# tphakala/birda

Hardware: AMD Instinct MI355X
Metric: 3s/48kHz segments/sec (BirdNET v2.4) (higher is better)
Workload: dtype f16x3; 1 GPU; configs[1]: 1000 synthetic 3 s/48 kHz segments per GPU per step, HBM-resident, seeded synthetic BirdNET-v2.4-shaped model (EfficientNet-B0-like, 6522 classes); segments_per_gpu=1000, micro_batch=1000, fused_blocks=16, precision=auto

## Files before the change

### birda_amd/csrc/api.hip

```cpp
#include "api_internal.hpp"
#include <unistd.h>
#include <cerrno>

namespace bhi {


thread_local std::string g_err;

int fail(int code, const char *fmt, ...) {
    char buf[1024];
    va_list ap;
    va_start(ap, fmt);
    vsnprintf(buf, sizeof buf, fmt, ap);
    va_end(ap);
    g_err = buf;
    if (code == BH_ERR_HIP) (void)hipGetLastError();
    return code;
}

int on_exception() noexcept {
    try { throw; }
    catch (const std::bad_alloc &) { return fail(BH_ERR_INTERNAL, "out of host memory"); }
    catch (const std::exception &e) { return fail(BH_ERR_INTERNAL, "internal error: %s", e.what()); }
    catch (...) { return fail(BH_ERR_INTERNAL, "internal error (unknown exception)"); }
// ... 923 lines not shown
        const uint32_t pf = cfg->flags & BH_FLAG_PRECISION_MASK;
        c->precision = pf == BH_FLAG_F32 ? 0 : pf == BH_FLAG_F16 ? 1 : 3;
        c->auto_fallback = pf == BH_FLAG_AUTO;
        c->low_latency = (cfg->flags & BH_FLAG_LOW_LATENCY) != 0;
        c->full_planes = (cfg->flags & BH_FLAG_FULL_PLANES) != 0;
        c->model_path = cfg->model_path;
    }
    if (const char *pe = (cfg->flags & FLAG_INTERNAL_NO_ENV) ? nullptr : getenv("BIRDA_HIP_PRECISION")) {
        if (!strcmp(pe, "f32")) { c->precision = 0; c->auto_fallback = false; }
        else if (!strcmp(pe, "f16x3")) { c->precision = 3; c->auto_fallback = false; }
        else if (!strcmp(pe, "auto")) { c->precision = 3; c->auto_fallback = true; }
        else if (!strcmp(pe, "f16")) { c->precision = 1; c->auto_fallback = false; }
        else return fail(BH_ERR_INVALID, "BIRDA_HIP_PRECISION must be auto, f32, f16x3 or f16");
    }
    int fe_prec = (c->precision != 0 && !(getenv("BIRDA_HIP_MEL_F32") && getenv("BIRDA_HIP_MEL_F32")[0] == '1')) ? 3 : 0;
    for (uint32_t b = 0; b < m.h.n_branches; b++)
        if (m.branches[b].frame_length % 256) fe_prec = 0;
    if (fe_prec == 3) {
        bool want = false, can = true;
        for (uint32_t b = 0; b < m.h.n_branches; b++) {
            if (m.branches[b].frame_step % 16 == 0) want = true;
            if (align_up(m.branches[b].n_mels, 16) % 32 || m.branches[b].frame_length % 512) can = false;
        }
        if (const char *e = getenv("BIRDA_HIP_MEL32")) want = e[0] == '1';
        if (want && can) fe_prec = 32;
    }
    if (m.h.sample_count % 4) return fail(BH_ERR_UNSUPPORTED, "front-end: sample_count %u must be a multiple of 4 (16-byte span loads)", m.h.sample_count);
    c->fe.prec = fe_prec;
    c->fe.n_branches = (int)m.h.n_branches;
    c->fe.sample_count = (int)m.h.sample_count;
    c->fe.norm_eps = m.h.norm_eps;
    for (uint32_t b = 0; b < m.h.n_branches; b++) {
        const auto &br = m.branches[b];
        const int nm_pad = (int)align_up(br.n_mels, 16);
        if (nm_pad < 32 || nm_pad > 128)
            return fail(BH_ERR_UNSUPPORTED, "front-end: n_mels %u not built (17 .. 128)", br.n_mels);
        if (b > 0 && nm_pad != c->fe.br[0].nm_pad) return fail(BH_ERR_UNSUPPORTED, "front-end: branches differ in n_mels");
        if (br.frame_length % 128 || br.fft_length != br.frame_length)
            return fail(BH_ERR_UNSUPPORTED, "front-end: frame_length %u must be a multiple of 128 and equal fft_length", br.frame_length);
        int gf_s = 0;
        std::vector<float> gf = build_gf(br, m.blob.data() + br.mel_w_off, nm_pad, fe_prec, &gf_s);
        float *d = nullptr;
        int rc = upload(gf.data(), gf.size() * sizeof(float), &d);
        if (rc != BH_OK) return rc;
        c->d_owned.push_back(d);
        auto &p = c->fe.br[b];
        p.gf = d; p.L = (int)br.frame_length; p.H = (int)br.frame_step; p.K = p.L / 2;
        p.n_mels = (int)br.n_mels; p.nm_pad = nm_pad; p.n_frames = (int)br.n_frames;
        p.expo = 1.0f / (1.0f + expf(br.mag_scale));
        p.log2_bias = -2.0f * (float)gf_s * p.expo;
        p.out_scale = br.out_scale; p.out_shift = br.out_shift; p.flip = (int)(br.flags & 1u);
        c->mel_flops += 2ull * (uint64_t)p.K * nm_pad * br.n_frames;
    }
    if (bh::mel_lds_bytes(c->fe) > 160 * 1024)
        return fail(BH_ERR_UNSUPPORTED, "front-end: a tile of frames at this hop and frame length spans %zu KB of samples, more than a CU's 160 KB of LDS",
                    bh::mel_lds_bytes(c->fe) / 1024);
    {
        float *d = nullptr;
        int rcf = upload(&c->fe, sizeof c->fe, &d);
        if (rcf != BH_OK) return rcf;
        c->d_fe = reinterpret_cast<bh::FrontendParams *>(d);
        c->d_owned.push_back(d);
    }
    int rc = upload(m.blob.data(), m.blob.size() * sizeof(float), &c->d_blob);
    if (rc != BH_OK) return rc;
    c->d_w.resize(m.layers.size());
    c->ldw.assign(m.layers.size(), 0);
    for (size_t i = 0; i < m.layers.size(); i++) {
        const auto &L = m.layers[i];
        c->d_w[i] = c->d_blob + L.w_off;
        if (L.op == bh::OP_PWCONV || L.op == bh::OP_DENSE) {
            if (L.cin % 4) return fail(BH_ERR_UNSUPPORTED, "layer %zu: cin %u not a multiple of 4", i, L.cin);
            const int ld = (int)align_up(L.cout, 4);
            c->ldw[i] = ld;
            if (ld != (int)L.cout) {
                const std::vector<float> w = pw_gemm_rows(m.blob.data() + L.w_off, L.cin, L.cout, (size_t)ld);
                float *d = nullptr;
                rc = upload(w.data(), w.size() * sizeof(float), &d);
                if (rc != BH_OK) return rc;
                c->d_owned.push_back(d);
                c->d_w[i] = d;
            }
        } else if (L.op == bh::OP_DWCONV) {
            if (!bh::dwconv_supports(conv_params(L)))
                return fail(BH_ERR_UNSUPPORTED, "layer %zu: depthwise %ux%u stride %u channels %u not built", i, L.kh, L.kw, L.sh, L.cout);
        } else if (L.op == bh::OP_CONV && L.in_layout == 1) {
            if (!bh::conv_direct_supports(conv_params(L)))
                return fail(BH_ERR_UNSUPPORTED, "layer %zu: direct conv shape not built", i);
        } else if (L.op == bh::OP_CONV) {
            const bh::ConvParams p = conv_params(L);
            if (!bh::conv_gemm_supports(p))
                return fail(BH_ERR_UNSUPPORTED, "layer %zu: full convolution %ux%u stride %ux%u, %u -> %u channels, layout %u not built "
                            "(kernel 1..7, stride 1 / 2, channels multiples of 4, NHWC)", i, L.kh, L.kw, L.sh, L.sw, L.cin, L.cout, L.in_layout);
            const int ld = (int)align_up(L.cout, 4);
            c->ldw[i] = ld;
            const std::vector<float> w = conv_gemm_rows(m.blob.data() + L.w_off, p, ld);
            float *d = nullptr;
            rc = upload(w.data(), w.size() * sizeof(float), &d);
            if (rc != BH_OK) return rc;
            c->d_owned.push_back(d);
            c->d_w[i] = d;
        } else if (L.op == bh::OP_GCONV) {
            const bh::ConvParams p = conv_params(L);
            if (!bh::gconv_supports(p, (int)L.reserved))
                return fail(BH_ERR_UNSUPPORTED, "layer %zu: grouped convolution %ux%u stride %ux%u, %u -> %u channels in %u groups not built "
                            "(kernel 1..7, stride 1 / 2, group widths multiples of 4, NHWC, no residual)", i, L.kh, L.kw, L.sh, L.sw, L.cin, L.cout, L.reserved);
// ... 1594 lines not shown
```

### birda_amd/csrc/kernels.hpp

```cpp
#pragma once
#include <hip/hip_runtime.h>
#include <stdint.h>

#include <atomic>
#include <cmath>
#include <mutex>

#ifdef BIRDA_HIP_EXPERIMENTS
#define BH_XENV(name) getenv(name)
#else
#define BH_XENV(name) (static_cast<const char *>(nullptr))
#endif

namespace bh {

constexpr int MAX_DEVICES = 64;
inline int current_device() {
    int d = 0;
    if (hipGetDevice(&d) != hipSuccess || d < 0 || d >= MAX_DEVICES) d = 0;
    return d;
}
struct DeviceOnce {
    std::mutex mu;
    std::atomic<unsigned char> done[MAX_DEVICES] = {};
// ... 203 lines not shown
__device__ __forceinline__ float bh_act(float v) {
    if constexpr (ACT == ACT_NONE) return v;
    else if constexpr (ACT == ACT_GELU_ERF) return gelu_erf_fast(v);
    else if constexpr (ACT == ACT_RELU) return bh_relu1(v);
    else if constexpr (ACT == ACT_RELU6) return __builtin_amdgcn_fmed3f(v, 0.0f, 6.0f);
    else if constexpr (ACT == ACT_SWISH) return v * __builtin_amdgcn_rcpf(1.0f + __builtin_amdgcn_exp2f(-1.4426950408889634f * v));
    else return act_apply_slow(v, ACT);
}
template <int ACT>
__device__ __forceinline__ bh_f32x2 bh_act2(bh_f32x2 v) {
    if constexpr (ACT == ACT_GELU_ERF) return gelu_erf_fast2(v);
    else { bh_f32x2 r; r[0] = bh_act<ACT>(v[0]); r[1] = bh_act<ACT>(v[1]); return r; }
}
template <int ACT>
__device__ __forceinline__ void bh_act4(bh_f32x2 &v0, bh_f32x2 &v1) {
    if constexpr (ACT == ACT_GELU_ERF) gelu_erf_fast4(v0, v1);
    else { v0 = bh_act2<ACT>(v0); v1 = bh_act2<ACT>(v1); }
}
inline bool act_is_templated(int act) { return act == ACT_GELU_ERF || act == ACT_SWISH || act == ACT_RELU6; }

__device__ __forceinline__ float bh_relu_keep_nan(float v) { return v < 0.0f ? 0.0f : v; }
__device__ __forceinline__ float bh_relu6_keep_nan(float v) { return v < 0.0f ? 0.0f : (v > 6.0f ? 6.0f : v); }
__device__ __forceinline__ float bh_act_limits(float v, float r) {
    r = v == __builtin_inff() ? v : r;
    return v == -__builtin_inff() ? 0.0f : r;
}
template <int ACT>
__device__ __forceinline__ float bh_act_after(float v) {
    if constexpr (ACT == ACT_RELU) return bh_relu_keep_nan(v);
    else if constexpr (ACT == ACT_RELU6) return bh_relu6_keep_nan(v);
    else return bh_act_limits(v, bh_act<ACT>(v));
}
__device__ __forceinline__ float act_apply_pos(float v, int act, bool after) {
    switch (act) {
    case ACT_RELU: return after ? bh_relu_keep_nan(v) : fmaxf(v, 0.f);
    case ACT_RELU6: return after ? bh_relu6_keep_nan(v) : fminf(fmaxf(v, 0.f), 6.f);
    case ACT_SWISH: { const float r = v / (1.0f + expf(-v)); return after ? bh_act_limits(v, r) : r; }
    case ACT_GELU_ERF: { const float r = gelu_erf_fast(v); return after ? bh_act_limits(v, r) : r; }
    case ACT_GELU_TANH: { const float r = 0.5f * v * (1.0f + tanhf(0.7978845608028654f * (v + 0.044715f * v * v * v))); return after ? bh_act_limits(v, r) : r; }
    case ACT_SIGMOID: return 1.0f / (1.0f + expf(-v));
    default: return v;
    }
}
inline bool act_is_templated_after(int act) { return act == ACT_RELU || act_is_templated(act); }

struct BranchParams {
    const float *gf;
    int L, H, K;
    int n_mels, nm_pad, n_frames;
    float expo;
    float out_scale, out_shift;
    int flip;
    float log2_bias;
};
struct FrontendParams {
    BranchParams br[MAX_BRANCHES];
    int prec;
    int n_branches;
    int sample_count;
    float norm_eps;
};

void launch_segment_pcm(const void *d_pcm_origin, int sample_format, size_t n_frames, int channels, const unsigned long long *d_starts,
                        int n_seg, int seg_len, float *d_out, size_t out_stride, hipStream_t s);
void launch_minmax(const float *x, float *minmax, unsigned *in_bad, int n_seg, int sample_count, hipStream_t s);
size_t mel_lds_bytes(const FrontendParams &p);
const char *launch_mel(const float *x, const float *minmax, float *spec, const FrontendParams &p,
                       const FrontendParams *d_p, int n_seg, hipStream_t s);


struct ConvParams {
    int in_h, in_w, out_h, out_w, cin, cout, kh, kw, sh, sw, pad_t, pad_l, in_layout, act;
    int res_after = 0;
};
bool conv_direct_supports(const ConvParams &p);
const char *launch_conv_direct(const float *in, const float *w, const float *b, float *out, const ConvParams &p,
                        int n_seg, hipStream_t s);
bool conv_gemm_supports(const ConvParams &p);
bool conv_gemm16_supports(const ConvParams &p);
bool conv_gemm16_after_supports(const ConvParams &p);
const char *launch_conv_gemm(const float *in, const float *W, const float *b, const float *R, float *out, const ConvParams &p, int n_seg,
                             int ldw, hipStream_t s);
const char *launch_conv_gemm16(const float *in, const void *Wf, const float *b, const float *R, float *out, const ConvParams &p, int n_seg,
                               int terms, float w_unscale, hipStream_t s);
__host__ __device__ inline void gconv_tile_span(int cin, int cout, int groups, int t, int &c0, int &span) {
    const int gi = cin / groups, go = cout / groups;
    const int last = (16 * t + 15 < cout ? 16 * t + 15 : cout - 1) / go, first = 16 * t / go;
    c0 = first * gi;
    span = (last - first + 1) * gi;
}
bool gconv_supports(const ConvParams &p, int groups);
const char *launch_gconv(const float *in, const float *Wf, const float *b, float *out, const ConvParams &p, int groups, int n_seg, hipStream_t s);
const char *launch_gconv16(const float *in, const void *Wf, const float *b, float *out, const ConvParams &p, int groups, int n_seg, int terms,
                           float w_unscale, hipStream_t s);
bool dwconv_supports(const ConvParams &p);
const char *launch_dwconv(const float *in, const float *w, const float *b, float *out, const ConvParams &p,
                   int n_seg, hipStream_t s);
const char *launch_pw_gemm(const float *A, const float *W, const float *bias, const float *R, float *C, int M, int K,
                          int N, int ldw, int act, hipStream_t s, int res_after = 0);
bool pw_gemm16_supports(int K, int act);
bool pw_gemm16_after_supports(int K, int act);
const char *launch_pw_gemm16(const float *A, const void *Wf, const float *bias, const float *R, float *C, int M, int K, int N,
                             int act, int terms, float w_unscale, hipStream_t s, int res_after = 0);
const char *launch_pw_gemm_gated(const float *A, const float *gate, int rows_per_seg, const float *W, const float *bias, const float *R,
                                 float *C, int M, int K, int N, int ldw, int act, hipStream_t s, int res_after = 0);
bool pw_gemm16_gated_wants_blocked(int K, int N, int rows_per_seg);
const char *launch_pw_gemm16_gated(const float *A, const float *gate, int rows_per_seg, const void *Wf, const float *bias, const float *R,
                                   float *C, int M, int K, int N, int terms, float w_unscale, int a_blocked, hipStream_t s);
bool se_gate16_supports(int C, int Cr);
const char *launch_se_gate16(const float *part, int tiles, int P, float *hpart, const float *W1, const float *b1, int ld1, int act1, const float *W2,
                      const float *b2, int ld2, int act2, float *gate, int n_seg, int C, int Cr, hipStream_t s);
bool se_gate_supports(int C, int Cr);
const char *launch_se_gate_gemm(const float *part, int tiles, int P, float *pooled, float *hidden, const float *W1, const float *b1, int ld1, int act1,
                         const float *W2, const float *b2, int ld2, int act2, float *gate, int n_seg, int C, int Cr, hipStream_t s);
const char *launch_se_gate(const float *part, int tiles, int P, const float *W1, const float *b1, int ld1, int act1, const float *W2, const float *b2,
                    int ld2, int act2, float *gate, int n_seg, int C, int Cr, hipStream_t s);
const char *launch_gap(const float *in, float *out, int n_seg, int P, int C, hipStream_t s);
const char *launch_scale(const float *in, const float *gate, float *out, int n_seg, int P, int C, hipStream_t s);
// ... 68 lines not shown
```

### birda_amd/csrc/kernels_frontend.hip

```cpp
#include <algorithm>
#include <cstdlib>

#include "kernels.hpp"

namespace bh {

constexpr int MM_SPLIT = 8;

typedef float f32x4 __attribute__((ext_vector_type(4)));
typedef _Float16 f16x8 __attribute__((ext_vector_type(8)));

__device__ inline float wave_min(float v) {
#pragma unroll
    for (int o = 32; o > 0; o >>= 1) v = fminf(v, __shfl_xor(v, o, 64));
    return v;
}
__device__ inline float wave_max(float v) {
#pragma unroll
    for (int o = 32; o > 0; o >>= 1) v = fmaxf(v, __shfl_xor(v, o, 64));
    return v;
}

__global__ __launch_bounds__(256) void minmax_kernel(const float *__restrict__ x, float *__restrict__ mm,
                                                      unsigned *__restrict__ in_bad, int sample_count) {
    const int seg = blockIdx.y, part = blockIdx.x;
    const int n4 = sample_count >> 2;
    const int per = (n4 + MM_SPLIT - 1) / MM_SPLIT;
    const int lo = part * per, hi = min(n4, lo + per);
    const float4 *p = reinterpret_cast<const float4 *>(x + (size_t)seg * sample_count);
    float mn = INFINITY, mx = -INFINITY;
    float z0 = 0.0f, z1 = 0.0f;
    for (int i = lo + threadIdx.x; i < hi; i += 256) {
        float4 v = p[i];
        mn = fminf(fminf(mn, v.x), fminf(v.y, fminf(v.z, v.w)));
        mx = fmaxf(fmaxf(mx, v.x), fmaxf(v.y, fmaxf(v.z, v.w)));
        z0 = __builtin_fmaf(v.x, 0.0f, z0); z1 = __builtin_fmaf(v.y, 0.0f, z1);
        z0 = __builtin_fmaf(v.z, 0.0f, z0); z1 = __builtin_fmaf(v.w, 0.0f, z1);
    }
    if (part == MM_SPLIT - 1)
        for (int i = (n4 << 2) + threadIdx.x; i < sample_count; i += 256) {
            float v = x[(size_t)seg * sample_count + i];
            mn = fminf(mn, v); mx = fmaxf(mx, v);
            z0 = __builtin_fmaf(v, 0.0f, z0);
        }
    mn = wave_min(mn); mx = wave_max(mx);
    const int any_bad = __syncthreads_or((z0 + z1) != 0.0f ? 1 : 0);
    __shared__ float s[8];
    const int w = threadIdx.x >> 6;
    if ((threadIdx.x & 63) == 0) { s[w] = mn; s[4 + w] = mx; }
    __syncthreads();
    if (threadIdx.x == 0) {
        mn = fminf(fminf(s[0], s[1]), fminf(s[2], s[3]));
        mx = fmaxf(fmaxf(s[4], s[5]), fmaxf(s[6], s[7]));
        mm[((size_t)seg * MM_SPLIT + part) * 2 + 0] = mn;
// ... 12 lines not shown
    else if constexpr (FMT == 2) {
        const int32_t v = (int32_t)((uint32_t)p[0] << 8 | (uint32_t)p[1] << 16 | (uint32_t)p[2] << 24);
        return (float)v / 2147483648.0f;
    } else if constexpr (FMT == 3) return (float)*reinterpret_cast<const int32_t *>(p) / 2147483648.0f;
    else return *reinterpret_cast<const float *>(p);
}

template <int FMT>
__global__ __launch_bounds__(256) void segment_pcm_kernel(const unsigned char *__restrict__ pcm, long n_frames, int channels,
                                                           const unsigned long long *__restrict__ starts,
                                                           int seg_len, float *__restrict__ out, long out_stride) {
    constexpr int BPS = FMT == 1 ? 2 : FMT == 2 ? 3 : 4;
    const int seg = blockIdx.y;
    const long s0 = (long)starts[seg];
    float *o = out + (long)seg * out_stride;
    for (int j = blockIdx.x * 256 + threadIdx.x; j < seg_len; j += gridDim.x * 256) {
        const long f = s0 + j;
        float v = 0.0f;
        if (f < n_frames) {
            if (channels == 1) {
                v = pcm_sample<FMT>(pcm + f * BPS);
            } else {
                float sum = 0.0f;
                for (int c = 0; c < channels; c++) sum += pcm_sample<FMT>(pcm + (f * channels + c) * BPS);
                v = sum / (float)channels;
            }
        }
        o[j] = v;
    }
}

void launch_segment_pcm(const void *d_pcm_origin, int sample_format, size_t n_frames, int channels, const unsigned long long *d_starts,
                        int n_seg, int seg_len, float *d_out, size_t out_stride, hipStream_t s) {
    dim3 grid((unsigned)std::min<size_t>(((size_t)seg_len + 255) / 256, 64), n_seg), block(256);
    const unsigned char *p = static_cast<const unsigned char *>(d_pcm_origin);
#define BH_SEG(F) hipLaunchKernelGGL(segment_pcm_kernel<F>, grid, block, 0, s, p, (long)n_frames, channels, d_starts, seg_len, d_out, (long)out_stride)
    switch (sample_format) {
    case 2: BH_SEG(2); break;
    case 3: BH_SEG(3); break;
    case 4: BH_SEG(4); break;
    default: BH_SEG(1); break;
    }
#undef BH_SEG
}

#ifndef BH_MEL_PIPE
#define BH_MEL_PIPE 2
#endif
#ifndef BH_MEL_GM
#define BH_MEL_GM 6
#define BH_MEL_GD 6
#define BH_MEL_GV 8
#endif
constexpr int MEL_FT = 3;
constexpr int MEL_TN = 16 * MEL_FT;


template <int MT, int PREC, int HALVES = 1>
__global__ __launch_bounds__(256 * HALVES, (MT <= 6 || HALVES == 2) ? 2 : 1) void mel_kernel(const float *__restrict__ x, const float *__restrict__ mm,
                                                      float *__restrict__ spec, const FrontendParams *__restrict__ pp,
                                                      const float *__restrict__ gf0, const float *__restrict__ gf1,
                                                      const float *__restrict__ gf2, const float *__restrict__ gf3,
                                                      const int dbg_arg, const int n_tiles, const int n_items, const int paired) {
    extern __shared__ __attribute__((aligned(16))) float smem[];
#ifdef BIRDA_HIP_EXPERIMENTS
    const int dbg = dbg_arg;
#else
    constexpr int dbg = 0; (void)dbg_arg;
#endif
    const int n_branches = pp->n_branches;
    const int S = pp->sample_count;
    float *xs = smem;
    const int tid = threadIdx.x, lane = tid & 63;
    const int half = HALVES == 2 ? tid >> 8 : 0, wave = (tid >> 6) & 3;
    const int li = lane & 15, kq = lane >> 4;
    constexpr int TNW = MEL_TN * HALVES, NTHR = 256 * HALVES;

    static_assert(MM_SPLIT == 8, "16 floats of min / max partials per segment");
    constexpr int MEL_SU = HALVES == 2 ? 14 : (MT <= 6 ? 15 : 16);
    float4 q[MEL_SU], mmq[4];
    const int pr_xcd = blockIdx.x & 7, pr_slot = blockIdx.x >> 3;
    const int pr_role = paired ? pr_slot % n_branches : 0, pr_q = (pr_slot / n_branches) * 8 + pr_xcd;
    const int pr_stride = (int)gridDim.x / n_branches, n_pairs = n_items / n_branches;
    struct MelItem { int sg, br, tl, ok; };
    auto decode = [&](int n) __attribute__((always_inline)) -> MelItem {
        MelItem r;
        if (paired) {
            const int P = pr_q + n * pr_stride;
            r.br = (pr_role + n) % n_branches;
            r.sg = P / n_tiles; r.tl = P - r.sg * n_tiles;
            r.ok = P < n_pairs;
        } else {
            const int it = (int)blockIdx.x + n * (int)gridDim.x;
            r.tl = it % n_tiles;
            const int sb = it / n_tiles;
            r.sg = sb / n_branches; r.br = sb - r.sg * n_branches;
            r.ok = it < n_items;
        }
        return r;
    };
    auto issue = [&](int sg, int br, int tl) __attribute__((always_inline)) {
        const int Hn = pp->br[br].H, Ln = pp->br[br].L;
        const int sp = ((TNW - 1) * Hn + Ln + 3) & ~3, g0 = tl * TNW * Hn;
        const float *xg = x + (size_t)sg * S;
        (void)sp;
#pragma unroll
        for (int u = 0; u < MEL_SU; u++) q[u] = *reinterpret_cast<const float4 *>(xg + min(g0 + tid * 4 + u * 4 * NTHR, S - 4));
        const float4 *mv = reinterpret_cast<const float4 *>(mm + (size_t)sg * MM_SPLIT * 2);
        mmq[0] = mv[0]; mmq[1] = mv[1]; mmq[2] = mv[2]; mmq[3] = mv[3];
    };
    int step_n = 0;
    MelItem cur = decode(0);
    if (cur.ok) issue(cur.sg, cur.br, cur.tl);

    while (cur.ok) {
    const int seg = cur.sg, branch = cur.br, tile = cur.tl;
    BranchParams bp = pp->br[branch];
    const float *__restrict__ gfp = branch == 0 ? gf0 : branch == 1 ? gf1 : branch == 2 ? gf2 : gf3;
    const int t0 = tile * TNW;
    const int L = bp.L, H = bp.H, K = bp.K;
    const int span = (TNW - 1) * H + L;
    const int span_pad = (span + 3) & ~3;

    const float mn = fminf(fminf(fminf(mmq[0].x, mmq[0].z), fminf(mmq[1].x, mmq[1].z)), fminf(fminf(mmq[2].x, mmq[2].z), fminf(mmq[3].x, mmq[3].z)));
    const float mx = fmaxf(fmaxf(fmaxf(mmq[0].y, mmq[0].w), fmaxf(mmq[1].y, mmq[1].w)), fmaxf(fmaxf(mmq[2].y, mmq[2].w), fmaxf(mmq[3].y, mmq[3].w)));
    const float sc = 2.0f / ((mx - mn) + pp->norm_eps);

    const float *xseg = x + (size_t)seg * S;
    const int g0s = t0 * H;
    if (g0s + span_pad <= S) {
#pragma unroll
        for (int u = 0; u < MEL_SU; u++) {
            const int i = tid * 4 + u * 4 * NTHR;
            if (i < span_pad) {
                float4 v = q[u];
                v.x = fmaf(v.x - mn, sc, -1.0f); v.y = fmaf(v.y - mn, sc, -1.0f);
                v.z = fmaf(v.z - mn, sc, -1.0f); v.w = fmaf(v.w - mn, sc, -1.0f);
                *reinterpret_cast<float4 *>(xs + i) = v;
            }
        }
    } else {
#pragma unroll
    for (int u = 0; u < MEL_SU; u++) {
        const int i = tid * 4 + u * 4 * NTHR;
        if (i < span_pad) {
            float4 v = q[u];
            v.x = (g0s + i + 0 < S) ? fmaf(v.x - mn, sc, -1.0f) : -1.0f;
            v.y = (g0s + i + 1 < S) ? fmaf(v.y - mn, sc, -1.0f) : -1.0f;
            v.z = (g0s + i + 2 < S) ? fmaf(v.z - mn, sc, -1.0f) : -1.0f;
            v.w = (g0s + i + 3 < S) ? fmaf(v.w - mn, sc, -1.0f) : -1.0f;
            *reinterpret_cast<float4 *>(xs + i) = v;
        }
    }
    }
    for (int i = MEL_SU * 4 * NTHR + tid * 4; i < span_pad; i += 4 * NTHR) {
        float4 v;
        v.x = (g0s + i + 0 < S) ? fmaf(xseg[g0s + i + 0] - mn, sc, -1.0f) : -1.0f;
        v.y = (g0s + i + 1 < S) ? fmaf(xseg[g0s + i + 1] - mn, sc, -1.0f) : -1.0f;
        v.z = (g0s + i + 2 < S) ? fmaf(xseg[g0s + i + 2] - mn, sc, -1.0f) : -1.0f;
        v.w = (g0s + i + 3 < S) ? fmaf(xseg[g0s + i + 3] - mn, sc, -1.0f) : -1.0f;
        *reinterpret_cast<float4 *>(xs + i) = v;
    }
    __syncthreads();

    f32x4 acc[MEL_FT][MT];
#pragma unroll
    for (int f = 0; f < MEL_FT; f++)
#pragma unroll
        for (int m = 0; m < MT; m++) acc[f][m] = (f32x4){0.f, 0.f, 0.f, 0.f};

    const int gpw = K / 64;
    const int gbeg = wave * gpw;
    const float4 *gA = reinterpret_cast<const float4 *>(gfp) + lane;
    if constexpr (PREC == 3) {
        const int spw = K / 128, sbeg = wave * spw;
        const f16x8 *gA = reinterpret_cast<const f16x8 *>(gfp) + lane;
        [[maybe_unused]] f16x8 a0h[MT], a0l[MT], a1h[MT], a1l[MT];
        [[maybe_unused]] auto load = [&](int st, f16x8 (&ah)[MT], f16x8 (&al)[MT]) {
            if (dbg & 16) st = sbeg;
#pragma unroll
            for (int m = 0; m < MT; m++) {
                ah[m] = gA[(((size_t)st * MT + m) * 2 + 0) * 64];
                al[m] = gA[(((size_t)st * MT + m) * 2 + 1) * 64];
            }
        };
        const float *xf = xs + (half * MEL_TN + li) * H;
        [[maybe_unused]] auto step = [&](int st, const f16x8 (&ah)[MT], const f16x8 (&al)[MT]) {
            const int j0 = st * 32 + kq;
            f16x8 bh[MEL_FT], bl[MEL_FT];
#pragma unroll
            for (int f = 0; f < MEL_FT; f++)
            {
                float y[8];
#pragma unroll
                for (int jj = 0; jj < 8; jj++)
                    y[jj] = bh_add_unpacked(xf[f * 16 * H + j0 + 4 * jj + 1], xf[f * 16 * H + L - 1 - j0 - 4 * jj]);
                bh_split8(y, bh[f], bl[f]);
            }
            __builtin_amdgcn_sched_barrier(0);
#pragma unroll
            for (int m = 0; m < MT; m++)
#pragma unroll
                for (int f = 0; f < MEL_FT; f++) {
                    acc[f][m] = __builtin_amdgcn_mfma_f32_16x16x32_f16(ah[m], bh[f], acc[f][m], 0, 0, 0);
                    acc[f][m] = __builtin_amdgcn_mfma_f32_16x16x32_f16(ah[m], bl[f], acc[f][m], 0, 0, 0);
                    acc[f][m] = __builtin_amdgcn_mfma_f32_16x16x32_f16(al[m], bh[f], acc[f][m], 0, 0, 0);
                }
        };
#if BH_MEL_PIPE == 1
        auto build = [&](int st, f16x8 (&bh)[MEL_FT], f16x8 (&bl)[MEL_FT]) {
            const int j0 = st * 32 + kq;
#pragma unroll
            for (int f = 0; f < MEL_FT; f++) {
                float y[8];
#pragma unroll
                for (int jj = 0; jj < 8; jj++)
                    y[jj] = bh_add_unpacked(xf[f * 16 * H + j0 + 4 * jj + 1], xf[f * 16 * H + L - 1 - j0 - 4 * jj]);
                bh_split8(y, bh[f], bl[f]);
            }
        };
        auto mma = [&](const f16x8 (&ah)[MT], const f16x8 (&al)[MT], const f16x8 (&bh)[MEL_FT], const f16x8 (&bl)[MEL_FT]) {
#pragma unroll
            for (int m = 0; m < MT; m++)
#pragma unroll
                for (int f = 0; f < MEL_FT; f++) {
                    acc[f][m] = __builtin_amdgcn_mfma_f32_16x16x32_f16(ah[m], bh[f], acc[f][m], 0, 0, 0);
                    acc[f][m] = __builtin_amdgcn_mfma_f32_16x16x32_f16(ah[m], bl[f], acc[f][m], 0, 0, 0);
                    acc[f][m] = __builtin_amdgcn_mfma_f32_16x16x32_f16(al[m], bh[f], acc[f][m], 0, 0, 0);
                }
        };
        auto interleave = [&]() {
#pragma unroll
            for (int g = 0; g < 9 * MT / BH_MEL_GM; g++) {
                __builtin_amdgcn_sched_group_barrier(0x008, BH_MEL_GM, 0);
                __builtin_amdgcn_sched_group_barrier(0x100, BH_MEL_GD, 0);
                __builtin_amdgcn_sched_group_barrier(0x002, BH_MEL_GV, 0);
            }
        };
        f16x8 b0h[MEL_FT], b0l[MEL_FT], b1h[MEL_FT], b1l[MEL_FT];
        load(sbeg, a0h, a0l);
        if (!(dbg & 1) && (HALVES == 1 || t0 + half * MEL_TN < bp.n_frames)) {
            build(sbeg, b0h, b0l);
            __builtin_amdgcn_sched_barrier(0);
            int si = 0;
            for (; si + 2 < spw; si += 2) {
                load(sbeg + si + 1, a1h, a1l);
                __builtin_amdgcn_sched_barrier(0);
                build(sbeg + si + 1, b1h, b1l);
                mma(a0h, a0l, b0h, b0l);
                interleave();
                __builtin_amdgcn_sched_barrier(0);
                load(sbeg + si + 2, a0h, a0l);
                __builtin_amdgcn_sched_barrier(0);
                build(sbeg + si + 2, b0h, b0l);
                mma(a1h, a1l, b1h, b1l);
                interleave();
                __builtin_amdgcn_sched_barrier(0);
            }
            if (si + 1 < spw) {
                load(sbeg + si + 1, a1h, a1l);
                __builtin_amdgcn_sched_barrier(0);
                build(sbeg + si + 1, b1h, b1l);
                mma(a0h, a0l, b0h, b0l);
                interleave();
                __builtin_amdgcn_sched_barrier(0);
                mma(a1h, a1l, b1h, b1l);
            } else {
                mma(a0h, a0l, b0h, b0l);
            }
        }
#elif BH_MEL_PIPE == 2
        #ifndef BH_MEL_FT1
#define BH_MEL_FT1 ((MEL_FT + 1) / 2)
#endif
        constexpr int MH = (MT + 1) / 2, FT1 = BH_MEL_FT1;
        f16x8 aLh[MH], aLl[MH], aHh[MH], aHl[MH];
        auto load_half = [&](int st, int h, f16x8 (&ah)[MH], f16x8 (&al)[MH]) {
            if (dbg & 16) st = sbeg;
#pragma unroll
            for (int m = 0; m < MH; m++) {
                if (h * MH + m >= MT) continue;
                ah[m] = gA[(((size_t)st * MT + h * MH + m) * 2 + 0) * 64];
                al[m] = gA[(((size_t)st * MT + h * MH + m) * 2 + 1) * 64];
            }
        };
        auto build_f = [&](int st, int f0, int f1, f16x8 (&bh)[MEL_FT], f16x8 (&bl)[MEL_FT]) {
            const int j0 = st * 32 + kq;
#pragma unroll
            for (int f = 0; f < MEL_FT; f++) {
                if (f < f0 || f >= f1) continue;
                float y[8];
#pragma unroll
                for (int jj = 0; jj < 8; jj++)
                    y[jj] = bh_add_unpacked(xf[f * 16 * H + j0 + 4 * jj + 1], xf[f * 16 * H + L - 1 - j0 - 4 * jj]);
                bh_split8(y, bh[f], bl[f]);
            }
        };
        auto mma_half = [&](int h, const f16x8 (&ah)[MH], const f16x8 (&al)[MH], const f16x8 (&bh)[MEL_FT], const f16x8 (&bl)[MEL_FT]) {
#pragma unroll
            for (int m = 0; m < MH; m++)
#pragma unroll
                for (int f = 0; f < MEL_FT; f++) {
                    if (h * MH + m >= MT) continue;
                    const int mm = h * MH + m < MT ? h * MH + m : 0;
                    acc[f][mm] = __builtin_amdgcn_mfma_f32_16x16x32_f16(ah[m], bh[f], acc[f][mm], 0, 0, 0);
                    acc[f][mm] = __builtin_amdgcn_mfma_f32_16x16x32_f16(ah[m], bl[f], acc[f][mm], 0, 0, 0);
                    acc[f][mm] = __builtin_amdgcn_mfma_f32_16x16x32_f16(al[m], bh[f], acc[f][mm], 0, 0, 0);
                }
        };
        auto interleave = [&](int nf) {
            constexpr int NM = 9 * MH;
            const int groups = NM / BH_MEL_GM;
#pragma unroll
            for (int g = 0; g < NM / BH_MEL_GM; g++) {
                __builtin_amdgcn_sched_group_barrier(0x008, BH_MEL_GM, 0);
                __builtin_amdgcn_sched_group_barrier(0x100, (16 * FT1 + NM / BH_MEL_GM - 1) / (NM / BH_MEL_GM), 0);
                __builtin_amdgcn_sched_group_barrier(0x002, (24 * FT1 + NM / BH_MEL_GM - 1) / (NM / BH_MEL_GM), 0);
            }
            (void)groups; (void)nf;
        };
        f16x8 b0h[MEL_FT], b0l[MEL_FT], b1h[MEL_FT], b1l[MEL_FT];
        load_half(sbeg, 0, aLh, aLl);
        load_half(sbeg, 1, aHh, aHl);
        if (!(dbg & 1) && (HALVES == 1 || t0 + half * MEL_TN < bp.n_frames)) {
            build_f(sbeg, 0, MEL_FT, b0h, b0l);
            __builtin_amdgcn_sched_barrier(0);
            auto one = [&](int st, const f16x8 (&ch)[MEL_FT], const f16x8 (&cl)[MEL_FT], f16x8 (&nh)[MEL_FT], f16x8 (&nl)[MEL_FT], bool more) __attribute__((always_inline)) {
                if (more) build_f(st + 1, 0, FT1, nh, nl);
                mma_half(0, aLh, aLl, ch, cl);
                if (more) interleave(FT1);
                __builtin_amdgcn_sched_barrier(0);
                if (more) load_half(st + 1, 0, aLh, aLl);
                __builtin_amdgcn_sched_barrier(0);
                if (more) build_f(st + 1, FT1, MEL_FT, nh, nl);
                mma_half(1, aHh, aHl, ch, cl);
                if (more) interleave(MEL_FT - FT1);
                __builtin_amdgcn_sched_barrier(0);
                if (more) load_half(st + 1, 1, aHh, aHl);
                __builtin_amdgcn_sched_barrier(0);
            };
            int si = 0;
            for (; si + 2 < spw; si += 2) {
                one(sbeg + si, b0h, b0l, b1h, b1l, true);
                one(sbeg + si + 1, b1h, b1l, b0h, b0l, true);
            }
            if (si + 1 < spw) {
                one(sbeg + si, b0h, b0l, b1h, b1l, true);
                one(sbeg + si + 1, b1h, b1l, b0h, b0l, false);
            } else {
                one(sbeg + si, b0h, b0l, b1h, b1l, false);
            }
        }
#else
        load(sbeg, a0h, a0l);
        if (!(dbg & 1) && (HALVES == 1 || t0 + half * MEL_TN < bp.n_frames)) {
            int si = 0;
            for (; si + 2 < spw; si += 2) {
                load(sbeg + si + 1, a1h, a1l);
                __builtin_amdgcn_sched_barrier(0);
                step(sbeg + si, a0h, a0l);
                __builtin_amdgcn_sched_barrier(0);
                load(sbeg + si + 2, a0h, a0l);
                __builtin_amdgcn_sched_barrier(0);
                step(sbeg + si + 1, a1h, a1l);
                __builtin_amdgcn_sched_barrier(0);
            }
            if (si + 1 < spw) {
                load(sbeg + si + 1, a1h, a1l);
                __builtin_amdgcn_sched_barrier(0);
                step(sbeg + si, a0h, a0l);
                __builtin_amdgcn_sched_barrier(0);
                step(sbeg + si + 1, a1h, a1l);
            } else {
                step(sbeg + si, a0h, a0l);
            }
        }
#endif
    } else {
    float4 a0[MT], a1[MT];
#pragma unroll
    for (int m = 0; m < MT; m++) a0[m] = gA[((size_t)gbeg * MT + m) * 64];

    const float *xf = xs + li * H;
    auto group = [&](int g, const float4 (&a)[MT]) {
        const int jb = g * 16 + 4 * kq;
        float b[4][MEL_FT];
#pragma unroll
        for (int c = 0; c < 4; c++)
#pragma unroll
            for (int f = 0; f < MEL_FT; f++)
                b[c][f] = xf[f * 16 * H + jb + c + 1] + xf[f * 16 * H + L - 1 - jb - c];
#pragma unroll
        for (int c = 0; c < 4; c++)
#pragma unroll
            for (int m = 0; m < MT; m++) {
                const float av = c == 0 ? a[m].x : c == 1 ? a[m].y : c == 2 ? a[m].z : a[m].w;
#pragma unroll
                for (int f = 0; f < MEL_FT; f++)
                    acc[f][m] = __builtin_amdgcn_mfma_f32_16x16x4f32(av, b[c][f], acc[f][m], 0, 0, 0);
            }
    };
    if (!(dbg & 1)) {
        int gi = 0;
        for (; gi + 2 < gpw; gi += 2) {
#pragma unroll
            for (int m = 0; m < MT; m++) a1[m] = gA[((size_t)(gbeg + gi + 1) * MT + m) * 64];
            __builtin_amdgcn_sched_barrier(0);
            group(gbeg + gi, a0);
            __builtin_amdgcn_sched_barrier(0);
#pragma unroll
            for (int m = 0; m < MT; m++) a0[m] = gA[((size_t)(gbeg + gi + 2) * MT + m) * 64];
            __builtin_amdgcn_sched_barrier(0);
            group(gbeg + gi + 1, a1);
            __builtin_amdgcn_sched_barrier(0);
        }
        if (gi + 1 < gpw) {
#pragma unroll
            for (int m = 0; m < MT; m++) a1[m] = gA[((size_t)(gbeg + gi + 1) * MT + m) * 64];
            __builtin_amdgcn_sched_barrier(0);
            group(gbeg + gi, a0);
            __builtin_amdgcn_sched_barrier(0);
            group(gbeg + gi + 1, a1);
        } else {
            group(gbeg + gi, a0);
        }
    }

    }
    const MelItem nxt = decode(step_n + 1);
    issue(nxt.ok ? nxt.sg : seg, nxt.ok ? nxt.br : branch, nxt.ok ? nxt.tl : tile);
// ... 171 lines not shown
                load(sc0 + 2, a0h, a0l);
                step(1, a1h, a1l);
                load(sc0 + 3, a1h, a1l);
                step(2, a0h, a0l);
                load(last ? sc0 + 3 : sc0 + 4, a0h, a0l);
                step(3, a1h, a1l);
                __builtin_amdgcn_fence(__ATOMIC_ACQ_REL, "wavefront");
                __builtin_amdgcn_wave_barrier();
                __builtin_amdgcn_sched_barrier(0);
            }
        }

        __syncthreads();
        float4 *red = reinterpret_cast<float4 *>(smem);
#pragma unroll
        for (int m = 0; m < MT32; m++)
#pragma unroll
            for (int r4 = 0; r4 < 4; r4++)
                red[((wave * MT32 + m) * 4 + r4) * 64 + lane] = make_float4(acc[m][4 * r4], acc[m][4 * r4 + 1], acc[m][4 * r4 + 2], acc[m][4 * r4 + 3]);
        __syncthreads();
        if (wave < MT32) {
            f32x16 tot;
#pragma unroll
            for (int r4 = 0; r4 < 4; r4++) {
                float4 v = red[((0 * MT32 + wave) * 4 + r4) * 64 + lane];
#pragma unroll
                for (int sw = 1; sw < 4; sw++) {
                    const float4 w = red[((sw * MT32 + wave) * 4 + r4) * 64 + lane];
                    v.x += w.x; v.y += w.y; v.z += w.z; v.w += w.w;
                }
                tot[4 * r4] = v.x; tot[4 * r4 + 1] = v.y; tot[4 * r4 + 2] = v.z; tot[4 * r4 + 3] = v.w;
            }
            const int t = t0 + fn;
            if (t < bp.n_frames) {
                float *out = spec + ((size_t)seg * n_branches + branch) * bp.n_mels * bp.n_frames;
#pragma unroll
                for (int r = 0; r < 16; r++) {
                    const int mel = 32 * wave + (r & 3) + 4 * kh + 8 * (r >> 2);
                    if (mel < bp.n_mels) {
                        const float v = tot[r];
                        float o = __builtin_amdgcn_exp2f(__builtin_fmaf(bp.expo, __builtin_amdgcn_logf(v * v), bp.log2_bias));
                        o = o * bp.out_scale + bp.out_shift;
                        const int row = bp.flip ? (bp.n_mels - 1 - mel) : mel;
                        out[(size_t)row * bp.n_frames + t] = o;
                    }
                }
            }
        }
        __syncthreads();
        item = next;
    }
}

size_t mel_lds_bytes(const FrontendParams &p) {
    int max_span = 0, span32 = 0;
    const int nmp = p.br[0].nm_pad;
    for (int b = 0; b < p.n_branches; b++) {
        max_span = std::max(max_span, (MEL_TN - 1) * p.br[b].H + p.br[b].L);
        span32 = std::max(span32, (MEL32_TN - 1) * p.br[b].H + p.br[b].L);
    }
    if (p.prec == 32)
        return std::max((size_t)(((span32 + 3) & ~3) + 4 * 2 * 32 * MEL32_YP) * sizeof(float), (size_t)4 * (nmp / 32) * 4 * 64 * sizeof(float4));
    return std::max((size_t)((max_span + 3) & ~3) * sizeof(float), (size_t)4 * 3 * (nmp / 16) * 64 * sizeof(float4));
}

const char *launch_mel(const float *x, const float *minmax, float *spec, const FrontendParams &p,
                       const FrontendParams *d_p, int n_seg, hipStream_t s) {
    int max_span = 0, max_frames = 0, nmp = p.br[0].nm_pad;
    for (int b = 0; b < p.n_branches; b++) {
        int span = (MEL_TN - 1) * p.br[b].H + p.br[b].L;
        max_span = span > max_span ? span : max_span;
        max_frames = p.br[b].n_frames > max_frames ? p.br[b].n_frames : max_frames;
    }
    static const int dbg = [] { const char *e = BH_XENV("BIRDA_HIP_MEL_DBG"); return e ? atoi(e) : 0; }();
    if (p.prec == 32) {
        int span32 = 0;
        for (int b = 0; b < p.n_branches; b++) span32 = std::max(span32, (MEL32_TN - 1) * p.br[b].H + p.br[b].L);
        const int mt32 = nmp / 32;
        const int ybuf_off = (span32 + 3) & ~3;
        const size_t smem32 = std::max((size_t)(ybuf_off + 4 * 2 * 32 * MEL32_YP) * sizeof(float), (size_t)4 * mt32 * 4 * 64 * sizeof(float4));
        const int nt32 = (max_frames + MEL32_TN - 1) / MEL32_TN, ni32 = nt32 * p.n_branches * n_seg;
        const int n_cu32 = device_cu_count();
        dim3 g32((unsigned)std::min(ni32, 2 * n_cu32)), b32(256);
#define BH_MEL32(MTV)                                                                                                          \
    case MTV: {                                                                                                                \
        static DeviceOnce set32;                                                                                               \
        set32.run([] { (void)hipFuncSetAttribute((const void *)mel32_kernel<MTV>, hipFuncAttributeMaxDynamicSharedMemorySize, 160 * 1024); }); \
        hipLaunchKernelGGL((mel32_kernel<MTV>), g32, b32, smem32, s, x, minmax, spec, d_p, p.br[0].gf, p.br[1].gf, p.br[2].gf, p.br[3].gf, dbg, ybuf_off, nt32, ni32); \
        return "bh::mel32_kernel<" #MTV ">";                                                                                   \
    }
        switch (mt32) {
            BH_MEL32(1)
            BH_MEL32(2)
            BH_MEL32(3)
            BH_MEL32(4)
        default: break;
        }
#undef BH_MEL32
        return nullptr;
    }
    const int mt = nmp / 16;
    static const bool halves_on = BH_XENV("BIRDA_HIP_MEL_HALVES") && BH_XENV("BIRDA_HIP_MEL_HALVES")[0] == '2';
    int max_span2 = 0;
    for (int b = 0; b < p.n_branches; b++) max_span2 = std::max(max_span2, (2 * MEL_TN - 1) * p.br[b].H + p.br[b].L);
    const bool two = halves_on && p.prec == 3 && mt == 6 && ((size_t)((max_span2 + 3) & ~3) * 4 <= 160 * 1024) && ((max_span2 + 3) & ~3) <= 14 * 2048;
    const int tnw = two ? 2 * MEL_TN : MEL_TN;
    const size_t span_bytes = (size_t)(((two ? max_span2 : max_span) + 3) & ~3) * sizeof(float);
    const size_t red_bytes = (size_t)(two ? 8 : 4) * 3 * mt * 64 * sizeof(float4);
    const size_t smem = span_bytes > red_bytes ? span_bytes : red_bytes;
    const int n_tiles = (max_frames + tnw - 1) / tnw, n_items = n_tiles * p.n_branches * n_seg;
    const int n_cu = device_cu_count();
    int n_wg = std::min(n_items, ((mt <= 6 && !two) ? 2 : 1) * n_cu);
    static const bool pair_off = BH_XENV("BIRDA_HIP_MEL_PAIR") && BH_XENV("BIRDA_HIP_MEL_PAIR")[0] == '0';
    const int pair_group = 8 * p.n_branches;
    const int paired = (!pair_off && p.n_branches > 1 && n_wg >= pair_group) ? 1 : 0;
    if (paired) n_wg -= n_wg % pair_group;
    dim3 grid((unsigned)n_wg), block(256);
#ifdef BIRDA_HIP_EXPERIMENTS
    if (two) {
        static DeviceOnce attr2;
        attr2.run([] { (void)hipFuncSetAttribute((const void *)mel_kernel<6, 3, 2>, hipFuncAttributeMaxDynamicSharedMemorySize, 160 * 1024); });
        hipLaunchKernelGGL((mel_kernel<6, 3, 2>), grid, dim3(512), smem, s, x, minmax, spec, d_p, p.br[0].gf, p.br[1].gf, p.br[2].gf, p.br[3].gf,
                           dbg, n_tiles, n_items, paired);
        return "bh::mel_kernel<6, 3, 2>";
    }
#endif
#define BH_MEL_CASE(MTV)                                                                                   \
    case MTV: {                                                                                            \
        static DeviceOnce attr_set;                                                                        \
        attr_set.run([] {                                                                                  \
            (void)hipFuncSetAttribute((const void *)mel_kernel<MTV, 0>, hipFuncAttributeMaxDynamicSharedMemorySize, \
                                160 * 1024);                                                              \
            (void)hipFuncSetAttribute((const void *)mel_kernel<MTV, 3>, hipFuncAttributeMaxDynamicSharedMemorySize, \
                                160 * 1024);                                                              \
        });                                                                                                \
        if (p.prec == 3) {                                                                                 \
            hipLaunchKernelGGL((mel_kernel<MTV, 3>), grid, block, smem, s, x, minmax, spec, d_p, p.br[0].gf,   \
                               p.br[1].gf, p.br[2].gf, p.br[3].gf, dbg, n_tiles, n_items, paired);                 \
            return "bh::mel_kernel<" #MTV ", 3, 1>";                                                       \
        }                                                                                                  \
        hipLaunchKernelGGL((mel_kernel<MTV, 0>), grid, block, smem, s, x, minmax, spec, d_p, p.br[0].gf,       \
                           p.br[1].gf, p.br[2].gf, p.br[3].gf, dbg, n_tiles, n_items, paired);                     \
        return "bh::mel_kernel<" #MTV ", 0, 1>";                                                           \
    }
    switch (mt) {
        BH_MEL_CASE(2)
        BH_MEL_CASE(3)
        BH_MEL_CASE(4)
        BH_MEL_CASE(5)
        BH_MEL_CASE(6)
        BH_MEL_CASE(7)
        BH_MEL_CASE(8)
    default: break;
    }
#undef BH_MEL_CASE
    return nullptr;
}

}
```

Measured before the change: 152,100 segments/s.

## Skew mel front-end LDS staging to avoid bank conflicts for 1024/280 geometry

```diff
diff --git a/birda_amd/csrc/api.hip b/birda_amd/csrc/api.hip
--- a/birda_amd/csrc/api.hip
+++ b/birda_amd/csrc/api.hip
@@ -999,6 +999,7 @@
         p.out_scale = br.out_scale; p.out_shift = br.out_shift; p.flip = (int)(br.flags & 1u);
         c->mel_flops += 2ull * (uint64_t)p.K * nm_pad * br.n_frames;
     }
+    bh::mel_assign_span_pads(c->fe);
     if (bh::mel_lds_bytes(c->fe) > 160 * 1024)
         return fail(BH_ERR_UNSUPPORTED, "front-end: a tile of frames at this hop and frame length spans %zu KB of samples, more than a CU's 160 KB of LDS",
                     bh::mel_lds_bytes(c->fe) / 1024);
diff --git a/birda_amd/csrc/kernels.hpp b/birda_amd/csrc/kernels.hpp
--- a/birda_amd/csrc/kernels.hpp
+++ b/birda_amd/csrc/kernels.hpp
@@ -279,7 +279,38 @@
     float out_scale, out_shift;
     int flip;
     float log2_bias;
-};
+    int pad;
+    unsigned rcp_h;
+};
+
+constexpr bool mel_stride_conflict_free(int S) {
+    unsigned seen = 0;
+    for (int e = 0; e < 2; e++)
+        for (int t = 0; t < 16; t++) {
+            const unsigned bit = 1u << ((S * t + e) & 31);
+            if (seen & bit) return false;
+            seen |= bit;
+        }
+    return true;
+}
+constexpr int mel_hop_pad(int H) {
+    if (H <= 0 || mel_stride_conflict_free(H) || H % 4) return 0;
+    for (int pad = 2; pad <= 6; pad += 2)
+        if (mel_stride_conflict_free(H + pad)) return pad;
+    return 0;
+}
+#define BH_MEL_SKEW_GEOMS(X) X(1024, 280)
+constexpr int mel_span_pad(int L, int H, int prec) {
+    if (prec != 3) return 0;
+#define BH_MEL_SKEW_MATCH(LV, HV) if (L == LV && H == HV) return mel_hop_pad(HV);
+    BH_MEL_SKEW_GEOMS(BH_MEL_SKEW_MATCH)
+#undef BH_MEL_SKEW_MATCH
+    return 0;
+}
+constexpr int mel_staged_floats(int L, int H, int pad, int frames) {
+    const int span4 = ((frames - 1) * H + L + 3) & ~3;
+    return ((span4 - 1) + (pad ? pad * ((span4 - 1) / H) : 0) + 1 + 3) & ~3;
+}
 struct FrontendParams {
     BranchParams br[MAX_BRANCHES];
     int prec;
@@ -291,6 +322,7 @@
 void launch_segment_pcm(const void *d_pcm_origin, int sample_format, size_t n_frames, int channels, const unsigned long long *d_starts,
                         int n_seg, int seg_len, float *d_out, size_t out_stride, hipStream_t s);
 void launch_minmax(const float *x, float *minmax, unsigned *in_bad, int n_seg, int sample_count, hipStream_t s);
+void mel_assign_span_pads(FrontendParams &p);
 size_t mel_lds_bytes(const FrontendParams &p);
 const char *launch_mel(const float *x, const float *minmax, float *spec, const FrontendParams &p,
                        const FrontendParams *d_p, int n_seg, hipStream_t s);
diff --git a/birda_amd/csrc/kernels_frontend.hip b/birda_amd/csrc/kernels_frontend.hip
--- a/birda_amd/csrc/kernels_frontend.hip
+++ b/birda_amd/csrc/kernels_frontend.hip
@@ -1,5 +1,6 @@
 #include <algorithm>
 #include <cstdlib>
+#include <type_traits>
 
 #include "kernels.hpp"
 
@@ -118,6 +119,12 @@
 #define BH_MEL_GD 6
 #define BH_MEL_GV 8
 #endif
+template <int L_, int H_, int PAD_>
+struct MelGeo {
+    static constexpr int L = L_, H = H_, PAD = PAD_, HP = H_ + PAD_;
+    static_assert(PAD_ == 0 || (H_ % 4 == 0 && L_ % 256 == 0 && H_ > 36), "a pad falls on a multiple of 4 and at most once within a 32-deep step");
+    static __host__ __device__ constexpr int g(int j) { return j + PAD_ * (j / (H_ ? H_ : 1)); }
+};
 constexpr int MEL_FT = 3;
 constexpr int MEL_TN = 16 * MEL_FT;
 
@@ -146,8 +153,9 @@
     constexpr int MEL_SU = HALVES == 2 ? 14 : (MT <= 6 ? 15 : 16);
     float4 q[MEL_SU], mmq[4];
     const int pr_xcd = blockIdx.x & 7, pr_slot = blockIdx.x >> 3;
-    const int pr_role = paired ? pr_slot % n_branches : 0, pr_q = (pr_slot / n_branches) * 8 + pr_xcd;
-    const int pr_stride = (int)gridDim.x / n_branches, n_pairs = n_items / n_branches;
+    const int pr_role = __builtin_amdgcn_readfirstlane(paired ? pr_slot % n_branches : 0);
+    const int pr_q = __builtin_amdgcn_readfirstlane((pr_slot / n_branches) * 8 + pr_xcd);
+    const int pr_stride = __builtin_amdgcn_readfirstlane((int)gridDim.x / n_branches), n_pairs = __builtin_amdgcn_readfirstlane(n_items / n_branches);
     struct MelItem { int sg, br, tl, ok; };
     auto decode = [&](int n) __attribute__((always_inline)) -> MelItem {
         MelItem r;
@@ -194,7 +202,34 @@
 
     const float *xseg = x + (size_t)seg * S;
     const int g0s = t0 * H;
-    if (g0s + span_pad <= S) {
+    const int pad = bp.pad;
+    auto put_skewed = [&](int i, const float4 &v) __attribute__((always_inline)) {
+        float2 *d = reinterpret_cast<float2 *>(xs + i + pad * (int)__umulhi((unsigned)i, bp.rcp_h));
+        d[0] = make_float2(v.x, v.y); d[1] = make_float2(v.z, v.w);
+    };
+    if (pad) {
+        auto stage_skewed = [&](auto inside_c) __attribute__((always_inline)) {
+#pragma unroll
+            for (int u = 0; u < MEL_SU; u++) {
+                const int i = tid * 4 + u * 4 * NTHR;
+                if (i < span_pad) {
+                    float4 v = q[u];
+                    if constexpr (decltype(inside_c)::value) {
+                        v.x = fmaf(v.x - mn, sc, -1.0f); v.y = fmaf(v.y - mn, sc, -1.0f);
+                        v.z = fmaf(v.z - mn, sc, -1.0f); v.w = fmaf(v.w - mn, sc, -1.0f);
+                    } else {
+                        v.x = (g0s + i + 0 < S) ? fmaf(v.x - mn, sc, -1.0f) : -1.0f;
+                        v.y = (g0s + i + 1 < S) ? fmaf(v.y - mn, sc, -1.0f) : -1.0f;
+                        v.z = (g0s + i + 2 < S) ? fmaf(v.z - mn, sc, -1.0f) : -1.0f;
+                        v.w = (g0s + i + 3 < S) ? fmaf(v.w - mn, sc, -1.0f) : -1.0f;
+                    }
+                    put_skewed(i, v);
+                }
+            }
+        };
+        if (g0s + span_pad <= S) stage_skewed(std::true_type{});
+        else stage_skewed(std::false_type{});
+    } else if (g0s + span_pad <= S) {
 #pragma unroll
         for (int u = 0; u < MEL_SU; u++) {
             const int i = tid * 4 + u * 4 * NTHR;
@@ -225,7 +260,8 @@
         v.y = (g0s + i + 1 < S) ? fmaf(xseg[g0s + i + 1] - mn, sc, -1.0f) : -1.0f;
         v.z = (g0s + i + 2 < S) ? fmaf(xseg[g0s + i + 2] - mn, sc, -1.0f) : -1.0f;
         v.w = (g0s + i + 3 < S) ? fmaf(xseg[g0s + i + 3] - mn, sc, -1.0f) : -1.0f;
-        *reinterpret_cast<float4 *>(xs + i) = v;
+        if (pad) put_skewed(i, v);
+        else *reinterpret_cast<float4 *>(xs + i) = v;
     }
     __syncthreads();
 
@@ -239,8 +275,9 @@
     const int gbeg = wave * gpw;
     const float4 *gA = reinterpret_cast<const float4 *>(gfp) + lane;
     if constexpr (PREC == 3) {
-        const int spw = K / 128, sbeg = wave * spw;
         const f16x8 *gA = reinterpret_cast<const f16x8 *>(gfp) + lane;
+        auto main_loop = [&](auto geo, const int sbeg, const int spw) __attribute__((always_inline)) {
+        using G = decltype(geo);
         [[maybe_unused]] f16x8 a0h[MT], a0l[MT], a1h[MT], a1l[MT];
         [[maybe_unused]] auto load = [&](int st, f16x8 (&ah)[MT], f16x8 (&al)[MT]) {
             if (dbg & 16) st = sbeg;
@@ -250,17 +287,33 @@
                 al[m] = gA[(((size_t)st * MT + m) * 2 + 1) * 64];
             }
         };
-        const float *xf = xs + (half * MEL_TN + li) * H;
+        int frame_dist = G::PAD ? G::HP : H;
+        if constexpr (G::PAD != 0) asm volatile("" : "+s"(frame_dist));
+        const float *xf = xs + (half * MEL_TN + li) * frame_dist;
+        [[maybe_unused]] const float *xfw = xf + kq, *xrv = xf - kq, *xsp = xf + kq + (kq == 3 ? G::PAD : 0);
+        auto fold8 = [&](int st, int f, float (&y)[8]) __attribute__((always_inline)) {
+            if constexpr (G::PAD == 0) {
+                const int j0 = st * 32 + kq;
+#pragma unroll
+                for (int jj = 0; jj < 8; jj++)
+                    y[jj] = bh_add_unpacked(xf[f * 16 * H + j0 + 4 * jj + 1], xf[f * 16 * H + L - 1 - j0 - 4 * jj]);
+            } else {
+#pragma unroll
+                for (int jj = 0; jj < 8; jj++) {
+                    const int b = st * 32 + 4 * jj;
+                    const int gfw = G::g(b + 1), grv = G::g(G::L - 4 - b);
+                    const float *pf = G::g(b + 4) != gfw + 3 ? xsp : xfw;
+                    y[jj] = bh_add_unpacked(pf[f * 16 * G::HP + gfw], xrv[f * 16 * G::HP + grv + 3]);
+                }
+            }
+        };
         [[maybe_unused]] auto step = [&](int st, const f16x8 (&ah)[MT], const f16x8 (&al)[MT]) {
-            const int j0 = st * 32 + kq;
             f16x8 bh[MEL_FT], bl[MEL_FT];
 #pragma unroll
             for (int f = 0; f < MEL_FT; f++)
             {
                 float y[8];
-#pragma unroll
-                for (int jj = 0; jj < 8; jj++)
-                    y[jj] = bh_add_unpacked(xf[f * 16 * H + j0 + 4 * jj + 1], xf[f * 16 * H + L - 1 - j0 - 4 * jj]);
+                fold8(st, f, y);
                 bh_split8(y, bh[f], bl[f]);
             }
             __builtin_amdgcn_sched_barrier(0);
@@ -275,13 +328,10 @@
         };
 #if BH_MEL_PIPE == 1
         auto build = [&](int st, f16x8 (&bh)[MEL_FT], f16x8 (&bl)[MEL_FT]) {
-            const int j0 = st * 32 + kq;
 #pragma unroll
             for (int f = 0; f < MEL_FT; f++) {
                 float y[8];
-#pragma unroll
-                for (int jj = 0; jj < 8; jj++)
-                    y[jj] = bh_add_unpacked(xf[f * 16 * H + j0 + 4 * jj + 1], xf[f * 16 * H + L - 1 - j0 - 4 * jj]);
+                fold8(st, f, y);
                 bh_split8(y, bh[f], bl[f]);
             }
         };
@@ -351,14 +401,11 @@
             }
         };
         auto build_f = [&](int st, int f0, int f1, f16x8 (&bh)[MEL_FT], f16x8 (&bl)[MEL_FT]) {
-            const int j0 = st * 32 + kq;
 #pragma unroll
             for (int f = 0; f < MEL_FT; f++) {
                 if (f < f0 || f >= f1) continue;
                 float y[8];
-#pragma unroll
-                for (int jj = 0; jj < 8; jj++)
-                    y[jj] = bh_add_unpacked(xf[f * 16 * H + j0 + 4 * jj + 1], xf[f * 16 * H + L - 1 - j0 - 4 * jj]);
+                fold8(st, f, y);
                 bh_split8(y, bh[f], bl[f]);
             }
         };
@@ -405,6 +452,13 @@
                 if (more) load_half(st + 1, 1, aHh, aHl);
                 __builtin_amdgcn_sched_barrier(0);
             };
+            if constexpr (G::PAD != 0) {
+#pragma unroll
+                for (int s = 0; s < G::L / 256; s++) {
+                    if (s & 1) one(sbeg + s, b1h, b1l, b0h, b0l, s + 1 < G::L / 256);
+                    else one(sbeg + s, b0h, b0l, b1h, b1l, s + 1 < G::L / 256);
+                }
+            } else {
             int si = 0;
             for (; si + 2 < spw; si += 2) {
                 one(sbeg + si, b0h, b0l, b1h, b1l, true);
@@ -415,6 +469,7 @@
                 one(sbeg + si + 1, b1h, b1l, b0h, b0l, false);
             } else {
                 one(sbeg + si, b0h, b0l, b1h, b1l, false);
+            }
             }
         }
 #else
@@ -442,6 +497,23 @@
             }
         }
 #endif
+        };
+        bool skewed = false;
+#define BH_MEL_SKEW_RUN(LV, HV)                                                                                     \
+        if (!skewed && pad && L == LV && H == HV) {                                                                \
+            using G = MelGeo<LV, HV, mel_hop_pad(HV)>;                                                             \
+            constexpr int SPW = LV / 256;                                                                          \
+            switch (__builtin_amdgcn_readfirstlane(wave)) {                                                        \
+            case 0: main_loop(G{}, 0, SPW); break;                                                                 \
+            case 1: main_loop(G{}, SPW, SPW); break;                                                               \
+            case 2: main_loop(G{}, 2 * SPW, SPW); break;                                                           \
+            default: main_loop(G{}, 3 * SPW, SPW); break;                                                          \
+            }                                                                                                      \
+            skewed = true;                                                                                         \
+        }
+        BH_MEL_SKEW_GEOMS(BH_MEL_SKEW_RUN)
+#undef BH_MEL_SKEW_RUN
+        if (!skewed) main_loop(MelGeo<0, 0, 0>{}, wave * (K / 128), K / 128);
     } else {
     float4 a0[MT], a1[MT];
 #pragma unroll
@@ -719,16 +791,30 @@
     }
 }
 
+static int mel_max_staged(const FrontendParams &p, int frames) {
+    int m = 0;
+    for (int b = 0; b < p.n_branches; b++) m = std::max(m, mel_staged_floats(p.br[b].L, p.br[b].H, p.br[b].pad, frames));
+    return m;
+}
+
+void mel_assign_span_pads(FrontendParams &p) {
+    for (int b = 0; b < p.n_branches; b++) {
+        p.br[b].pad = 0;
+        p.br[b].rcp_h = p.br[b].H > 1 ? (unsigned)((0x100000000ull + (unsigned)p.br[b].H - 1) / (unsigned)p.br[b].H) : 0u;
+    }
+    const size_t plain = mel_lds_bytes(p);
+    for (int b = 0; b < p.n_branches; b++) p.br[b].pad = mel_span_pad(p.br[b].L, p.br[b].H, p.prec);
+    if (plain <= 80 * 1024 && mel_lds_bytes(p) > 80 * 1024)
+        for (int b = 0; b < p.n_branches; b++) p.br[b].pad = 0;
+}
+
 size_t mel_lds_bytes(const FrontendParams &p) {
-    int max_span = 0, span32 = 0;
+    int span32 = 0;
     const int nmp = p.br[0].nm_pad;
-    for (int b = 0; b < p.n_branches; b++) {
-        max_span = std::max(max_span, (MEL_TN - 1) * p.br[b].H + p.br[b].L);
-        span32 = std::max(span32, (MEL32_TN - 1) * p.br[b].H + p.br[b].L);
-    }
+    for (int b = 0; b < p.n_branches; b++) span32 = std::max(span32, (MEL32_TN - 1) * p.br[b].H + p.br[b].L);
     if (p.prec == 32)
         return std::max((size_t)(((span32 + 3) & ~3) + 4 * 2 * 32 * MEL32_YP) * sizeof(float), (size_t)4 * (nmp / 32) * 4 * 64 * sizeof(float4));
-    return std::max((size_t)((max_span + 3) & ~3) * sizeof(float), (size_t)4 * 3 * (nmp / 16) * 64 * sizeof(float4));
+    return std::max((size_t)mel_max_staged(p, MEL_TN) * sizeof(float), (size_t)4 * 3 * (nmp / 16) * 64 * sizeof(float4));
 }
 
 const char *launch_mel(const float *x, const float *minmax, float *spec, const FrontendParams &p,
@@ -772,7 +858,10 @@
     for (int b = 0; b < p.n_branches; b++) max_span2 = std::max(max_span2, (2 * MEL_TN - 1) * p.br[b].H + p.br[b].L);
     const bool two = halves_on && p.prec == 3 && mt == 6 && ((size_t)((max_span2 + 3) & ~3) * 4 <= 160 * 1024) && ((max_span2 + 3) & ~3) <= 14 * 2048;
     const int tnw = two ? 2 * MEL_TN : MEL_TN;
-    const size_t span_bytes = (size_t)(((two ? max_span2 : max_span) + 3) & ~3) * sizeof(float);
+    for (int b = 0; b < p.n_branches; b++)
+        if (p.br[b].pad != 0 && p.br[b].pad != mel_span_pad(p.br[b].L, p.br[b].H, p.prec)) return nullptr;
+    const size_t span_bytes = (size_t)mel_max_staged(p, tnw) * sizeof(float);
+    if (!two && (size_t)(((max_span + 3) & ~3)) * sizeof(float) <= 80 * 1024 && span_bytes > 80 * 1024) return nullptr;
     const size_t red_bytes = (size_t)(two ? 8 : 4) * 3 * mt * 64 * sizeof(float4);
     const size_t smem = span_bytes > red_bytes ? span_bytes : red_bytes;
     const int n_tiles = (max_frames + tnw - 1) / tnw, n_items = n_tiles * p.n_branches * n_seg;
```

Result: slower. 142,900 segments/s (-6.1%).
